# diff7/tts-king

Measured on AMD Instinct MI355X. Metric: FS2 train mel-frames/sec/GPU + HiFi-GAN RTF (22.05 kHz), batch=16, higher is better.
Workload: dtype bf16

## Files before the change

### tts_king_amd/csrc/batchnorm.hip

```cpp
#include "common.h"

namespace {

struct BnCommon {
  const void* x;
  const float* mean;
  const float* rstd;
  const float* gamma;
  const float* beta;
  const uint64_t* rng;
  int rows, C, use_tanh;
  float p;
  unsigned site;
  int x_f32;
  const int* frame_limit;
  int seg_len;
  uint8_t* keep;
  const long long* lens;
};
__device__ __forceinline__ float tanh_fast(float x) { return 1.f - 2.f * __frcp_rn(__expf(2.f * x) + 1.f); }
__device__ __forceinline__ bool bn_live(const int* frame_limit, int seg_len, int r) {
  return !frame_limit || (r % seg_len) < frame_limit[0];
}
__device__ __forceinline__ int bn_rows(const int* frame_limit, int seg_len, int rows) {
// ... 204 lines not shown
  if (blockIdx.x == 0 && dgamma)
    for (int c = threadIdx.x; c < a.C; c += 256) {
      dbeta[c] = accumulate ? dbeta[c] + sums[c] : sums[c];
      dgamma[c] = accumulate ? dgamma[c] + sums[a.C + c] : sums[a.C + c];
    }
  for (int64_t i = blockIdx.x * 256 + threadIdx.x; i < n; i += (int64_t)gridDim.x * 256) {
    const int r = (int)(i / tpr), c4 = (int)(i - (int64_t)r * tpr) * 4;
    float xh[4], dy[4];
    bn_dy(a, dout, dout_f32, r, c4, i, thr, scale, xh, dy);
    const f32x4 g = *(const f32x4*)(a.gamma + c4), rs = *(const f32x4*)(a.rstd + c4);
    const f32x4 s1 = *(const f32x4*)(sums + c4), s2 = *(const f32x4*)(sums + a.C + c4);
    float o[4];
#pragma unroll
    for (int e = 0; e < 4; ++e) o[e] = g[e] * rs[e] * (dy[e] - s1[e] * inv_n - xh[e] * s2[e] * inv_n);
    if (!bn_live(a.frame_limit, a.seg_len, r)) o[0] = o[1] = o[2] = o[3] = 0.f;
    *(uint2*)(dx + (int64_t)r * a.C + c4) = make_uint2(pack_bf2(o[0], o[1]), pack_bf2(o[2], o[3]));
  }
}


constexpr int BN_MAX_CHUNKS = 64;
__host__ __device__ inline int bn_slab(int C) { return (C % 64 == 0) ? 64 : C; }

struct BnSlab {
  int c0, slab, tpr, rpi, r_in, cq, rb, re;
  __device__ BnSlab(int C, int rows) {
    slab = bn_slab(C);
    c0 = blockIdx.x * slab;
    tpr = slab >> 2;
    rpi = 256 / tpr;
    r_in = threadIdx.x / tpr;
    cq = threadIdx.x % tpr;
    const int per = (rows + gridDim.y - 1) / gridDim.y;
    rb = blockIdx.y * per;
    re = min(rb + per, rows);
  }
};

__device__ __forceinline__ void bn_slab_store(const BnSlab& g, int C, const float s[4], const float q[4], float* red, float* partials) {
  if (g.r_in < g.rpi) {
#pragma unroll
    for (int e = 0; e < 4; ++e) { red[g.r_in * g.slab + g.cq * 4 + e] = s[e]; red[(g.rpi + g.r_in) * g.slab + g.cq * 4 + e] = q[e]; }
  }
  __syncthreads();
  for (int v = threadIdx.x; v < 2 * g.slab; v += 256) {
    const int half = v >= g.slab, c = v - half * g.slab;
    float acc = 0.f;
    for (int k = 0; k < g.rpi; ++k) acc += red[(half * g.rpi + k) * g.slab + c];
    partials[(int64_t)blockIdx.y * 2 * C + half * C + g.c0 + c] = acc;
  }
}

constexpr int BN_TOT = 256 + 1024;
__device__ __forceinline__ void bn_slab_totals(const float* __restrict__ partials, int nblk, int C, int c0, int slab, double* tot ) {
  const int nq = slab >> 1, groups = 256 / nq;
  const int t = threadIdx.x;
  if (t < groups * nq) {
    const int q = t % nq, g0 = t / nq;
    const int v0 = q * 4;
    const int col = v0 < slab ? c0 + v0 : C + c0 + (v0 - slab);
    double a[4] = {0.0, 0.0, 0.0, 0.0};
    for (int b = g0; b < nblk; b += 16 * groups) {
      f32x4 f[16];
#pragma unroll
      for (int u = 0; u < 16; ++u) {
        const int bb = b + u * groups;
        f[u] = *(const f32x4*)(partials + (int64_t)min(bb, nblk - 1) * 2 * C + col);
        if (bb >= nblk) f[u] = f32x4{0.f, 0.f, 0.f, 0.f};
      }
#pragma unroll
      for (int u = 0; u < 16; ++u)
#pragma unroll
        for (int e = 0; e < 4; ++e) a[e] += f[u][e];
    }
#pragma unroll
    for (int e = 0; e < 4; ++e) tot[256 + t * 4 + e] = a[e];
  }
  __syncthreads();
  if (t < 2 * slab) {
    double sum = 0.0;
    for (int k = 0; k < groups; ++k) sum += tot[256 + (k * nq + (t >> 2)) * 4 + (t & 3)];
    tot[t] = sum;
  }
  __syncthreads();
}

__global__ __launch_bounds__(256) void bn_stats2_kernel(const void* __restrict__ x, int x_f32, int rows, int C, float* __restrict__ partials,
                                                        const int* __restrict__ frame_limit, int seg_len) {
  extern __shared__ float red[];
  const BnSlab g(C, rows);
  const int c4 = g.c0 + g.cq * 4;
  float s[4] = {0, 0, 0, 0}, q[4] = {0, 0, 0, 0};
  if (g.r_in < g.rpi)
    for (int r0 = g.rb + g.r_in; r0 < g.re; r0 += 8 * g.rpi) {
      float v[8][4];
#pragma unroll
      for (int u = 0; u < 8; ++u) {
        const int r = r0 + u * g.rpi, rc = min(r, g.re - 1);
        ldx4(x, x_f32, (int64_t)rc * C + c4, v[u]);
        if (r >= g.re || !bn_live(frame_limit, seg_len, rc)) v[u][0] = v[u][1] = v[u][2] = v[u][3] = 0.f;
      }
#pragma unroll
      for (int u = 0; u < 8; ++u)
#pragma unroll
        for (int e = 0; e < 4; ++e) { s[e] += v[u][e]; q[e] += v[u][e] * v[u][e]; }
    }
  bn_slab_store(g, C, s, q, red, partials);
}

struct BnTrain {
  const float* partials;
  int nblk;
  float eps, momentum;
  float* mean;
  float* rstd;
  float* run_mean;
  float* run_var;
  long long* nbt;
};

template <bool RESID>
__global__ __launch_bounds__(256, RESID ? 3 : 4) void bn_apply2_kernel(const BnCommon a, const BnTrain t, const float* __restrict__ resid,
                                                        bf16_t* __restrict__ out16, float* __restrict__ out32) {
  __shared__ double tot[BN_TOT];
  __shared__ float ms[128], rs[128];
  const BnSlab g(a.C, a.rows);
  const int cl = g.cq * 4, c4 = g.c0 + cl, tprC = a.C >> 2;
  const bool act = g.r_in < g.rpi;
  float v[4][4], rr[RESID ? 4 : 1][4];
  bool live[4];
#pragma unroll
  for (int u = 0; u < 4; ++u) {
    const int r = g.rb + g.r_in + u * g.rpi, rc = max(min(r, g.re - 1), 0);
    live[u] = act && r < g.re && bn_live(a.frame_limit, a.seg_len, r);
    if (act) {
      ldx4(a.x, a.x_f32, (int64_t)rc * a.C + c4, v[u]);
      if constexpr (RESID) { const f32x4 q = *(const f32x4*)(resid + (int64_t)rc * a.C + c4); rr[u][0] = q[0]; rr[u][1] = q[1]; rr[u][2] = q[2]; rr[u][3] = q[3]; }
    }
  }
  f32x4 gm = f32x4{0.f, 0.f, 0.f, 0.f}, bt = gm;
  if (act) { gm = *(const f32x4*)(a.gamma + c4); bt = *(const f32x4*)(a.beta + c4); }
  bn_slab_totals(t.partials, t.nblk, a.C, g.c0, g.slab, tot);
  if ((int)threadIdx.x < g.slab) {
    const int c = threadIdx.x;
    const int n = bn_rows(a.frame_limit, a.seg_len, a.rows);
    const double m = tot[c] / n;
    double var = tot[g.slab + c] / n - m * m;
    if (var < 0.0) var = 0.0;
    ms[c] = (float)m;
    rs[c] = (float)(1.0 / sqrt(var + (double)t.eps));
    if (blockIdx.y == 0) {
      t.mean[g.c0 + c] = ms[c];
      t.rstd[g.c0 + c] = rs[c];
      if (t.run_mean) {
        t.run_mean[g.c0 + c] = (1.f - t.momentum) * t.run_mean[g.c0 + c] + t.momentum * (float)m;
        t.run_var[g.c0 + c] = (1.f - t.momentum) * t.run_var[g.c0 + c] + t.momentum * (float)(var * n / (n > 1 ? n - 1 : 1));
      }
      if (blockIdx.x == 0 && c == 0 && t.nbt) t.nbt[0] += 1;
    }
  }
  __syncthreads();
  if (!act) return;
  const unsigned thr = keep_threshold(a.p);
  const float scale = a.p > 0.f ? 1.f / (1.f - a.p) : 1.f;
#pragma unroll
  for (int u = 0; u < 4; ++u) {
    const int r = g.rb + g.r_in + u * g.rpi;
    if (r >= g.re) break;
    const int64_t i = (int64_t)r * tprC + (c4 >> 2);
    if (!live[u]) {
      if (out16) *(uint2*)(out16 + (int64_t)r * a.C + c4) = make_uint2(0u, 0u);
      if (out32) *(f32x4*)(out32 + (int64_t)r * a.C + c4) = f32x4{0.f, 0.f, 0.f, 0.f};
      if (a.keep) a.keep[i] = 0;
      continue;
    }
#pragma unroll
    for (int e = 0; e < 4; ++e) {
      v[u][e] = (v[u][e] - ms[cl + e]) * rs[cl + e] * gm[e] + bt[e];
      if (a.use_tanh) v[u][e] = tanh_fast(v[u][e]);
    }
    if (a.p > 0.f) {
      const unsigned nib = bn_keep4(a.rng, a.site, (unsigned)i, thr);
      drop4(v[u], nib, scale);
      if (a.keep) a.keep[i] = (uint8_t)nib;
    }
    if constexpr (RESID) {
#pragma unroll
      for (int e = 0; e < 4; ++e) v[u][e] += rr[u][e];
    }
    if (out16) *(uint2*)(out16 + (int64_t)r * a.C + c4) = make_uint2(pack_bf2(v[u][0], v[u][1]), pack_bf2(v[u][2], v[u][3]));
    if (out32) *(f32x4*)(out32 + (int64_t)r * a.C + c4) = f32x4{v[u][0], v[u][1], v[u][2], v[u][3]};
  }
}

__global__ __launch_bounds__(256) void bn_bwd_stats2_kernel(const BnCommon a, const void* __restrict__ dout, int dout_f32,
                                                            float* __restrict__ partials) {
  extern __shared__ float red[];
  const BnSlab g(a.C, a.rows);
  const int c4 = g.c0 + g.cq * 4, tprC = a.C >> 2;
  const unsigned thr = keep_threshold(a.p);
  const float scale = a.p > 0.f ? 1.f / (1.f - a.p) : 1.f;
  float s[4] = {0, 0, 0, 0}, q[4] = {0, 0, 0, 0};
  if (g.r_in < g.rpi)
    for (int r0 = g.rb + g.r_in; r0 < g.re; r0 += 8 * g.rpi) {
      float xh[8][4], dy[8][4];
#pragma unroll
      for (int u = 0; u < 8; ++u) {
        const int r = r0 + u * g.rpi, rc = min(r, g.re - 1);
        bn_dy(a, dout, dout_f32, rc, c4, (int64_t)rc * tprC + (c4 >> 2), thr, scale, xh[u], dy[u]);
        if (r >= g.re) { xh[u][0] = xh[u][1] = xh[u][2] = xh[u][3] = 0.f; dy[u][0] = dy[u][1] = dy[u][2] = dy[u][3] = 0.f; }
      }
#pragma unroll
      for (int u = 0; u < 8; ++u)
#pragma unroll
        for (int e = 0; e < 4; ++e) { s[e] += dy[u][e]; q[e] += dy[u][e] * xh[u][e]; }
    }
  bn_slab_store(g, a.C, s, q, red, partials);
}

__global__ __launch_bounds__(256, 4) void bn_bwd_apply2_kernel(const BnCommon a, const void* __restrict__ dout, int dout_f32,
                                                            const float* __restrict__ partials, int nblk, bf16_t* __restrict__ dx,
                                                            float* __restrict__ dgamma, float* __restrict__ dbeta, int accumulate) {
  __shared__ double tot[BN_TOT];
  __shared__ float s1s[128], s2s[128];
  const BnSlab g(a.C, a.rows);
  const int cl = g.cq * 4, c4 = g.c0 + cl, tprC = a.C >> 2;
  const bool act = g.r_in < g.rpi;
  const unsigned thr = keep_threshold(a.p);
  const float scale = a.p > 0.f ? 1.f / (1.f - a.p) : 1.f;
  float xh[4][4], dy[4][4];
#pragma unroll
  for (int u = 0; u < 4; ++u) {
    const int rc = max(min(g.rb + g.r_in + u * g.rpi, g.re - 1), 0);
    if (act) bn_dy(a, dout, dout_f32, rc, c4, (int64_t)rc * tprC + (c4 >> 2), thr, scale, xh[u], dy[u]);
  }
  bn_slab_totals(partials, nblk, a.C, g.c0, g.slab, tot);
  if ((int)threadIdx.x < g.slab) {
    const int c = threadIdx.x;
    s1s[c] = (float)tot[c];
    s2s[c] = (float)tot[g.slab + c];
    if (blockIdx.y == 0 && dgamma) {
      dbeta[g.c0 + c] = accumulate ? dbeta[g.c0 + c] + s1s[c] : s1s[c];
      dgamma[g.c0 + c] = accumulate ? dgamma[g.c0 + c] + s2s[c] : s2s[c];
    }
  }
  __syncthreads();
  if (!act) return;
  const float inv_n = 1.f / bn_rows(a.frame_limit, a.seg_len, a.rows);
  const f32x4 gm = *(const f32x4*)(a.gamma + c4), rsd = *(const f32x4*)(a.rstd + c4);
#pragma unroll
  for (int u = 0; u < 4; ++u) {
    const int r = g.rb + g.r_in + u * g.rpi;
    if (r >= g.re) break;
    float o[4];
#pragma unroll
    for (int e = 0; e < 4; ++e) o[e] = gm[e] * rsd[e] * (dy[u][e] - s1s[cl + e] * inv_n - xh[u][e] * s2s[cl + e] * inv_n);
    if (!bn_live(a.frame_limit, a.seg_len, r)) o[0] = o[1] = o[2] = o[3] = 0.f;
    *(uint2*)(dx + (int64_t)r * a.C + c4) = make_uint2(pack_bf2(o[0], o[1]), pack_bf2(o[2], o[3]));
  }
}

inline int bn_chunks(int rows) { int n = (rows + 15) / 16; return n > BN_MAX_CHUNKS ? BN_MAX_CHUNKS : (n < 1 ? 1 : n); }
inline int bn_apply_chunks(int rows, int C) { const int rpi = 256 / (bn_slab(C) >> 2); int n = (rows + 4 * rpi - 1) / (4 * rpi); return n < 1 ? 1 : n; }

inline int bn_blocks(int rows) { int n = (rows + 15) / 16; return n > 1024 ? 1024 : (n < 1 ? 1 : n); }

}

extern "C" int ttsk_bn_nblocks(int rows) { return bn_blocks(rows); }

static int bn_check(int rows, int C) {
  TTSK_REQUIRE(rows > 0 && C >= 4 && C <= 1024 && (C & 3) == 0, "batchnorm: C must be a multiple of 4, <= 1024 (got %d)", C);
  return 0;
}

static int limit_check(const int32_t* frame_limit, int seg_len, int rows) {
  TTSK_REQUIRE(!frame_limit || (seg_len > 0 && rows % seg_len == 0), "batchnorm: frame_limit needs rows %% seg_len == 0");
  return 0;
}

extern "C" int ttsk_bn_stats(const void* x, int x_is_f32, int rows, int C, float* partials, const int32_t* frame_limit, int seg_len,
                             void* stream) {
  TTSK_REQUIRE(x && partials, "bn_stats: null pointer");
  if (int rc = limit_check(frame_limit, seg_len, rows)) return rc;
  if (int rc = bn_check(rows, C)) return rc;
  const int rpi = 256 / (C >> 2);
  hipLaunchKernelGGL(bn_stats_kernel, dim3(bn_blocks(rows)), dim3(256), 2 * rpi * C * sizeof(float), (hipStream_t)stream,
                     x, x_is_f32, rows, C, partials, frame_limit, seg_len > 0 ? seg_len : 1);
  TTSK_CHECK_LAUNCH();
  return TTSK_OK;
}

extern "C" int ttsk_bn_finalize(const float* partials, int nblk, int C, int rows, float eps, float momentum, float* mean,
                                float* rstd, float* running_mean, float* running_var, int64_t* num_batches_tracked,
                                const int32_t* frame_limit, int seg_len, void* stream) {
  if (int rc = limit_check(frame_limit, seg_len, rows)) return rc;
  TTSK_REQUIRE(partials && mean && rstd && nblk > 0, "bn_finalize: null pointer");
  TTSK_REQUIRE((running_mean == nullptr) == (running_var == nullptr), "bn_finalize: running stats come in pairs");
  hipLaunchKernelGGL(bn_finalize_kernel, dim3((C + 15) / 16), dim3(256), 0, (hipStream_t)stream, partials, nblk, C, rows, eps,
                     momentum, mean, rstd, running_mean, running_var, (long long*)num_batches_tracked, frame_limit, seg_len > 0 ? seg_len : 1);
  TTSK_CHECK_LAUNCH();
  return TTSK_OK;
}

extern "C" int ttsk_rsqrt_eps(const float* var, float eps, float* rstd, int n, void* stream) {
  TTSK_REQUIRE(var && rstd && n > 0, "rsqrt_eps: bad arguments");
  hipLaunchKernelGGL(rsqrt_eps_kernel, dim3((n + 255) / 256), dim3(256), 0, (hipStream_t)stream, var, eps, rstd, n);
  TTSK_CHECK_LAUNCH();
  return TTSK_OK;
}
// ... 20 lines not shown
  TTSK_REQUIRE(x && mean && rstd && gamma && beta && lens && (out_bf16 || out_f32), "bn_apply_lens: null pointer");
  TTSK_REQUIRE(seg_len > 0 && rows % seg_len == 0, "bn_apply_lens: rows %% seg_len != 0");
  if (int rc = bn_check(rows, C)) return rc;
  BnCommon a{x, mean, rstd, gamma, beta, nullptr, rows, C, use_tanh, 0.f, 0u, x_is_f32, nullptr, seg_len, nullptr, (const long long*)lens};
  int64_t n = (int64_t)rows * (C >> 2);
  int blocks = (int)((n + 255) / 256);
  if (blocks > 4096) blocks = 4096;
  hipLaunchKernelGGL(bn_apply_kernel<true>, dim3(blocks), dim3(256), 0, (hipStream_t)stream, a, resid_f32, (bf16_t*)out_bf16, out_f32);
  TTSK_CHECK_LAUNCH();
  return TTSK_OK;
}

extern "C" int ttsk_bn_bwd_stats(const void* dout, int dout_is_f32, const void* x, int x_is_f32, const float* mean, const float* rstd,
                                 const float* gamma, const float* beta, int rows, int C, int use_tanh, float p, uint32_t site,
                                 const uint64_t* rng, float* partials, const int32_t* frame_limit, int seg_len, void* stream) {
  if (int rc = limit_check(frame_limit, seg_len, rows)) return rc;
  TTSK_REQUIRE(dout && x && mean && rstd && gamma && beta && partials, "bn_bwd_stats: null pointer");
  TTSK_REQUIRE(p == 0.f || rng, "bn_bwd_stats: dropout needs rng");
  if (int rc = bn_check(rows, C)) return rc;
  BnCommon a{x, mean, rstd, gamma, beta, rng, rows, C, use_tanh, p, site, x_is_f32, frame_limit, seg_len > 0 ? seg_len : 1};
  const int rpi = 256 / (C >> 2);
  hipLaunchKernelGGL(bn_bwd_stats_kernel, dim3(bn_blocks(rows)), dim3(256), 2 * rpi * C * sizeof(float), (hipStream_t)stream, a,
                     dout, dout_is_f32, partials);
  TTSK_CHECK_LAUNCH();
  return TTSK_OK;
}

extern "C" int ttsk_bn_bwd_apply(const void* dout, int dout_is_f32, const void* x, int x_is_f32, const float* mean, const float* rstd,
                                 const float* gamma, const float* beta, int rows, int C, int use_tanh, float p, uint32_t site,
                                 const uint64_t* rng, const float* sums, void* dx_bf16, float* dgamma, float* dbeta, int accumulate,
                                 const int32_t* frame_limit, int seg_len, void* stream) {
  if (int rc = limit_check(frame_limit, seg_len, rows)) return rc;
  TTSK_REQUIRE(dout && x && mean && rstd && gamma && beta && sums && dx_bf16, "bn_bwd_apply: null pointer");
  TTSK_REQUIRE((dgamma == nullptr) == (dbeta == nullptr), "bn_bwd_apply: dgamma/dbeta come in pairs");
  if (int rc = bn_check(rows, C)) return rc;
  BnCommon a{x, mean, rstd, gamma, beta, rng, rows, C, use_tanh, p, site, x_is_f32, frame_limit, seg_len > 0 ? seg_len : 1};
  int64_t n = (int64_t)rows * (C >> 2);
  int blocks = (int)((n + 255) / 256);
  if (blocks > 4096) blocks = 4096;
  hipLaunchKernelGGL(bn_bwd_apply_kernel, dim3(blocks), dim3(256), 0, (hipStream_t)stream, a, dout, dout_is_f32, sums,
                     (bf16_t*)dx_bf16, dgamma, dbeta, accumulate);
  TTSK_CHECK_LAUNCH();
  return TTSK_OK;
}

static int bn2_check(int rows, int C) {
  if (int rc = bn_check(rows, C)) return rc;
  TTSK_REQUIRE(C % 64 == 0 || C <= 128, "batchnorm (slab path): C must be a multiple of 64 or <= 128 (got %d)", C);
  return 0;
}

extern "C" int ttsk_bn_nchunks(int rows) { return bn_chunks(rows); }

extern "C" int ttsk_bn_stats_slab(const void* x, int x_is_f32, int rows, int C, float* partials, const int32_t* frame_limit, int seg_len,
                                  void* stream) {
  TTSK_REQUIRE(x && partials, "bn_stats_slab: null pointer");
  if (int rc = limit_check(frame_limit, seg_len, rows)) return rc;
  if (int rc = bn2_check(rows, C)) return rc;
  const int slab = bn_slab(C), rpi = 256 / (slab >> 2);
  hipLaunchKernelGGL(bn_stats2_kernel, dim3(C / slab, bn_chunks(rows)), dim3(256), 2 * rpi * slab * sizeof(float), (hipStream_t)stream,
                     x, x_is_f32, rows, C, partials, frame_limit, seg_len > 0 ? seg_len : 1);
  TTSK_CHECK_LAUNCH();
  return TTSK_OK;
}

extern "C" int ttsk_bn_train_apply(const void* x, int x_is_f32, const float* partials, int nblk, float eps, float momentum, float* mean,
                                   float* rstd, float* running_mean, float* running_var, int64_t* num_batches_tracked,
                                   const float* gamma, const float* beta, int rows, int C, int use_tanh, float p, uint32_t site,
                                   const uint64_t* rng, const float* resid_f32, void* out_bf16, float* out_f32, uint8_t* keep_out,
                                   const int32_t* frame_limit, int seg_len, void* stream) {
  if (int rc = limit_check(frame_limit, seg_len, rows)) return rc;
  TTSK_REQUIRE(x && partials && nblk > 0 && mean && rstd && gamma && beta && (out_bf16 || out_f32), "bn_train_apply: null pointer");
  TTSK_REQUIRE((running_mean == nullptr) == (running_var == nullptr), "bn_train_apply: running stats come in pairs");
  TTSK_REQUIRE(p == 0.f || rng, "bn_train_apply: dropout needs rng");
  if (int rc = bn2_check(rows, C)) return rc;
  BnCommon a{x, nullptr, nullptr, gamma, beta, rng, rows, C, use_tanh, p, site, x_is_f32, frame_limit, seg_len > 0 ? seg_len : 1, keep_out};
  BnTrain t{partials, nblk, eps, momentum, mean, rstd, running_mean, running_var, (long long*)num_batches_tracked};
  const dim3 grid(C / bn_slab(C), bn_apply_chunks(rows, C));
  if (resid_f32) hipLaunchKernelGGL(bn_apply2_kernel<true>, grid, dim3(256), 0, (hipStream_t)stream, a, t, resid_f32, (bf16_t*)out_bf16, out_f32);
  else hipLaunchKernelGGL(bn_apply2_kernel<false>, grid, dim3(256), 0, (hipStream_t)stream, a, t, resid_f32, (bf16_t*)out_bf16, out_f32);
  TTSK_CHECK_LAUNCH();
  return TTSK_OK;
}

extern "C" int ttsk_bn_bwd_stats_slab(const void* dout, int dout_is_f32, const void* x, int x_is_f32, const float* mean, const float* rstd,
                                      const float* gamma, const float* beta, int rows, int C, int use_tanh, float p, uint32_t site,
                                      const uint64_t* rng, const uint8_t* keep, float* partials, const int32_t* frame_limit, int seg_len,
                                      void* stream) {
  if (int rc = limit_check(frame_limit, seg_len, rows)) return rc;
  TTSK_REQUIRE(dout && x && mean && rstd && gamma && beta && partials, "bn_bwd_stats_slab: null pointer");
  TTSK_REQUIRE(p == 0.f || rng || keep, "bn_bwd_stats_slab: dropout needs rng or the forward's keep bits");
  if (int rc = bn2_check(rows, C)) return rc;
  BnCommon a{x, mean, rstd, gamma, beta, rng, rows, C, use_tanh, p, site, x_is_f32, frame_limit, seg_len > 0 ? seg_len : 1, (uint8_t*)keep};
  const int slab = bn_slab(C), rpi = 256 / (slab >> 2);
  hipLaunchKernelGGL(bn_bwd_stats2_kernel, dim3(C / slab, bn_chunks(rows)), dim3(256), 2 * rpi * slab * sizeof(float), (hipStream_t)stream,
                     a, dout, dout_is_f32, partials);
  TTSK_CHECK_LAUNCH();
  return TTSK_OK;
}

extern "C" int ttsk_bn_bwd_apply_slab(const void* dout, int dout_is_f32, const void* x, int x_is_f32, const float* mean, const float* rstd,
                                      const float* gamma, const float* beta, int rows, int C, int use_tanh, float p, uint32_t site,
                                      const uint64_t* rng, const uint8_t* keep, const float* partials, int nblk, void* dx_bf16, float* dgamma,
                                      float* dbeta, int accumulate, const int32_t* frame_limit, int seg_len, void* stream) {
  if (int rc = limit_check(frame_limit, seg_len, rows)) return rc;
  TTSK_REQUIRE(dout && x && mean && rstd && gamma && beta && partials && nblk > 0 && dx_bf16, "bn_bwd_apply_slab: null pointer");
  TTSK_REQUIRE((dgamma == nullptr) == (dbeta == nullptr), "bn_bwd_apply_slab: dgamma/dbeta come in pairs");
  TTSK_REQUIRE(p == 0.f || rng || keep, "bn_bwd_apply_slab: dropout needs rng or the forward's keep bits");
  if (int rc = bn2_check(rows, C)) return rc;
  BnCommon a{x, mean, rstd, gamma, beta, rng, rows, C, use_tanh, p, site, x_is_f32, frame_limit, seg_len > 0 ? seg_len : 1, (uint8_t*)keep};
  hipLaunchKernelGGL(bn_bwd_apply2_kernel, dim3(C / bn_slab(C), bn_apply_chunks(rows, C)), dim3(256), 0, (hipStream_t)stream, a, dout,
                     dout_is_f32, partials, nblk, (bf16_t*)dx_bf16, dgamma, dbeta, accumulate);
  TTSK_CHECK_LAUNCH();
  return TTSK_OK;
}
```

### tts_king_amd/csrc/ffn_conv.hip

```cpp
#include "common.h"
#include "tapring.h"

namespace {

constexpr int WC_H = 4, WC_NW = 8, WC_NT = WC_NW * 64, WC_KH = 4, WC_CT = 2, WC_COUT = WC_NW * WC_CT * 16;

struct WcArgs {
  const bf16_t* x;
  const bf16_t* w;
  const float* bias;
  void* out;
  int S, K, Cout, relu;
  int B, tiles_per_utt;
  const bf16_t* gate;
  int nsplit, ldx;
  int64_t out_split;
  const float* o32;
  float* delta;
  float* stats;
  const int* frame_limit;
  int ups_cout;
  int ups_half;
  const float* bnb_x;
  const float* bnb_mean;
// ... 136 lines not shown
  {
    const int id = blockIdx.x, ncg = (a.Cout / COUT) * a.nsplit, ntile = a.tiles_per_utt * a.B;
    const int xcd = id & 7, per = 8 / (ncg < 8 ? ncg : 8);
    int tile;
    if ((8 % (ncg < 8 ? ncg : 8)) == 0 && ncg <= 8 && (ntile * ncg) % 8 == 0 && ntile % per == 0) {
      cg = xcd / per;
      tile = (id >> 3) * per + (xcd % per);
    } else if (ncg % 8 == 0) {
      const int gpx = ncg >> 3, slot = id >> 3;
      tile = slot / gpx;
      cg = xcd * gpx + (slot - tile * gpx);
    } else {
      cg = id / ntile;
      tile = id - cg * ntile;
    }
    bi = tile / a.tiles_per_utt;
    t0 = (tile - bi * a.tiles_per_utt) * TT;
    sp = cg % a.nsplit;
    cg = cg / a.nsplit;
  }
  WC_STAMP(0);
  const int S = a.S, K = a.K, HK = (K - 1) / 2, NS = NP * K;
  const int ldx = a.ldx;
  const bf16_t* __restrict__ xb = a.x + (int64_t)bi * S * ldx + sp * C;
  const bf16_t* __restrict__ wbase = a.w;
  const int ks_total = (ldx + 31) / 32, ks_base = sp * (C / 32);
  const int cin_valid = a.cin_valid > 0 ? a.cin_valid : C;

  const __amdgpu_buffer_rsrc_t wres = weights_rsrc(wbase, K * ks_total * 32 * a.Cout * 2);
  const int wlane = PACKED ? (cg * (COUT / 16) + wave * CT) * 1024 + lane * 16 : ((cg * COUT + wave * CT * 16 + l15) * K * C + q * 8) * 2;
  constexpr bool CAN_DIRECT = PACKED && !F16 && CIN == 256 && TT == 112 && NWV == 8 && CTV == 2;
  const bool direct = CAN_DIRECT && a.direct;
  int wl[CT];
#pragma unroll
  for (int cc = 0; cc < CT; ++cc) {
    const int co = 32 * wave + 8 * (l15 >> 2) + 4 * cc + (l15 & 3);
    wl[cc] = direct ? (cg * (COUT / 16) + (co >> 4)) * 1024 + ((co & 15) + 16 * q) * 16 : wlane + cc * 1024;
  }
  const int kstep_bytes = (a.Cout / 16) * 1024;
  bf16x8 wa[KH][CT], wb[KH][CT], wc[KH][CT];
  auto load_w = [&](int g, bf16x8 (&w)[KH][CT]) __attribute__((always_inline)) {
    const int tap = g / NP, part = g - tap * NP;
    if (PACKED) {
      frags_load<KH, CT>(w, wres, wl, (tap * ks_total + ks_base + part * KH) * kstep_bytes, kstep_bytes);
    } else {
      const int soff = (tap * C + part * (KH * 32)) * 2;
#pragma unroll
      for (int ks = 0; ks < KH; ++ks)
#pragma unroll
        for (int cc = 0; cc < CT; ++cc) w[ks][cc] = frag_load(wres, wlane, soff + ks * 64 + cc * (16 * K * C * 2));
    }
  };

  {
    constexpr int NCH = (XROWS * CH8 + NT - 1) / NT;
    uint4 xv[NCH];
#pragma unroll
    for (int it = 0; it < NCH; ++it) {
      const int idx = it * NT + tid;
      const int row = idx / CH8, ch = idx - row * CH8;
      const int t = t0 - WC_H + row;
      xv[it] = make_uint4(0, 0, 0, 0);
      if (idx < XROWS * CH8 && t >= 0 && t < S && ch * 8 < cin_valid) xv[it] = *(const uint4*)(xb + (int64_t)t * ldx + ch * 8);
    }
    load_w(0, wa);
    if (!F16 || 1 < NS) load_w(min(1, NS - 1), wb);
    if (!F16 || 2 < NS) load_w(min(2, NS - 1), wc);
#pragma unroll
    for (int it = 0; it < NCH; ++it) {
      const int idx = it * NT + tid;
      const int row = idx / CH8, ch = idx - row * CH8;
      if (idx < XROWS * CH8) *(uint4*)(XW + row * RS + ch * 16) = xv[it];
    }
  }
  f32x4 bv[CT];
#pragma unroll
  for (int cc = 0; cc < CT; ++cc)
    bv[cc] = a.bias ? *(const f32x4*)(a.bias + cg * COUT + (direct ? 32 * wave + 8 * q + 4 * cc : (wave * CT + cc) * 16 + q * 4)) : f32x4{0.f, 0.f, 0.f, 0.f};
  WC_STAMP(1);
  __syncthreads();
  WC_STAMP(2);

  f32x4 acc[CT][NF];
#pragma unroll
  for (int cc = 0; cc < CT; ++cc)
#pragma unroll
    for (int i = 0; i < NF; ++i) acc[cc][i] = f32x4{0.f, 0.f, 0.f, 0.f};
  {
    const int inl = (l15 + WC_H) * RS + q * 16;
    const int ups_shift = F16 && a.ups_cout ? ((cg * COUT + wave * CT * 16) / a.ups_cout < a.ups_half ? -1 : 1) : 0;
    constexpr bool RING = NF <= 8;
    auto inp_of = [&](int g) __attribute__((always_inline)) {
      const int tap = g / NP, part = g - tap * NP;
      return inl + (F16 && a.ups_cout ? tap * ups_shift : tap - HK) * RS + part * (KH * 64);
    };
    bf16x8 ring[RING ? NF : 1];
    if constexpr (RING) ring_prime<NF, RS>(ring, XW, inp_of(0));
    auto step = [&](int g, const bf16x8 (&w)[KH][CT]) __attribute__((always_inline)) {
      const int inp = inp_of(g);
      if constexpr (RING) {
        tap_ring<F16, KH, CT, NF, RS>(acc, ring, w, XW, inp, inp_of(g + 1 < NS ? g + 1 : g));
      } else {
#pragma unroll
        for (int ks = 0; ks < KH; ++ks) {
#pragma unroll
          for (int i = 0; i < NF; ++i) {
            const bf16x8 Bf = *(const bf16x8*)(XW + inp + i * 16 * RS + ks * 64);
#pragma unroll
            for (int cc = 0; cc < CT; ++cc) acc[cc][i] = mfma16<F16>(w[ks][cc], Bf, acc[cc][i]);
          }
        }
      }
    };
    constexpr bool UNCOND = !F16;
#pragma unroll 1
    for (int g = 0; g < NS; g += 3) {
      step(g, wa);
      if (UNCOND || g + 3 < NS) load_w(min(g + 3, NS - 1), wa);
      if (g + 1 < NS) step(g + 1, wb);
      if (UNCOND || g + 4 < NS) load_w(min(g + 4, NS - 1), wb);
      if (g + 2 < NS) step(g + 2, wc);
      if (UNCOND || g + 5 < NS) load_w(min(g + 5, NS - 1), wc);
    }
  }
  WC_STAMP(3);
#ifdef TTSK_STAMPS
  if (a.stamps && lane == 0 && wave < 8) {
    a.stamps[(int64_t)blockIdx.x * 24 + 8 + wave] = __builtin_amdgcn_s_memrealtime();
    a.stamps[(int64_t)blockIdx.x * 24 + 16 + wave] = __builtin_amdgcn_s_getreg(63492);
  }
#endif
// ... 548 lines not shown
```

### tts_king_amd/csrc/layernorm.hip

```cpp
#include "common.h"
#include "proj32.h"

namespace {

constexpr int MAXJ = 4;

struct LnArgs {
  const bf16_t* y;
  const bf16_t* res;
  const float* gamma;
  const float* beta;
  bf16_t* out;
  bf16_t* z_save;
  float* mean;
  float* rstd;
  const long long* lens;
  const uint64_t* rng;
  const float* head_w;
  const float* head_b;
  float* head_out;
  int rows, D, seg_len;
  float p_pre, p_post, eps;
  unsigned site_pre, site_post;
  int group_rows;
// ... 229 lines not shown
  }
  const int nq = head ? 4 : 3;
  float* P = a.partials + (int64_t)blockIdx.x * (nq * D + (head ? 1 : 0));
  for (int qn = 0; qn < nq; ++qn) {
#pragma unroll
    for (int j = 0; j < MJ; ++j)
      if (j < nj)
#pragma unroll
        for (int e = 0; e < 4; ++e) {
          const float v = qn == 0 ? dbias[j][e] : qn == 1 ? dg[j][e] : qn == 2 ? db[j][e] : dhw[j][e];
          red[wave][j * 256 + lane * 4 + e] = v;
        }
    __syncthreads();
    for (int c = threadIdx.x; c < D; c += LNB_WAVES * 64) {
      float t = 0.f;
#pragma unroll
      for (int w = 0; w < LNB_WAVES; ++w) t += red[w][c];
      P[qn * D + c] = t;
    }
    __syncthreads();
  }
  if (head) {
    dhb = wave_sum(dhb);
    if (lane == 0) redb[wave] = dhb;
    __syncthreads();
    if (threadIdx.x == 0) {
      float t = 0.f;
#pragma unroll
      for (int w = 0; w < LNB_WAVES; ++w) t += redb[w];
      P[nq * D] = t;
    }
  }
}

__device__ __forceinline__ void unpack8(uint4 u, float* v) {
  v[0] = __uint_as_float(u.x << 16); v[1] = __uint_as_float(u.x & 0xFFFF0000u);
  v[2] = __uint_as_float(u.y << 16); v[3] = __uint_as_float(u.y & 0xFFFF0000u);
  v[4] = __uint_as_float(u.z << 16); v[5] = __uint_as_float(u.z & 0xFFFF0000u);
  v[6] = __uint_as_float(u.w << 16); v[7] = __uint_as_float(u.w & 0xFFFF0000u);
}
__device__ __forceinline__ uint4 pack8f(const float* v) {
  return make_uint4(pack_bf2(v[0], v[1]), pack_bf2(v[2], v[3]), pack_bf2(v[4], v[5]), pack_bf2(v[6], v[7]));
}
__device__ __forceinline__ void hold(uint4& v) { asm volatile("" : "+v"(v.x), "+v"(v.y), "+v"(v.z), "+v"(v.w)); }
__device__ __forceinline__ void hold(f32x4& v) { asm volatile("" : "+v"(v)); }
__device__ __forceinline__ void hold(float& v) { asm volatile("" : "+v"(v)); }
__device__ __forceinline__ float group16_sum(float v) { return quad16_sum(v); }

__device__ __forceinline__ void lnb256_row(const LnBwdArgs& a, int row, int c0, const float gam[16], uint64_t seed, uint64_t step,
                                           unsigned thr, float dscale, float sbias[16], float sgam[16], float sbeta[16], float dzv[16],
                                           const float* dl = nullptr ) {
  constexpr int D = 256;
  const bool live = row < a.rows;
  bool masked = !live;
  if (live && a.lens) { const int b = row / a.seg_len, t = row - b * a.seg_len; masked = t >= a.lens[b]; }
  float zz[16], d[16];
#pragma unroll
  for (int e = 0; e < 16; ++e) { zz[e] = 0.f; d[e] = 0.f; }
  const bool slabbed = dl || a.slabs, use = live && !masked;
  const int64_t ro = (int64_t)(live ? row : a.rows - 1) * D + c0;
  uint4 zr[2] = {*(const uint4*)(a.z + ro), *(const uint4*)(a.z + ro + 8)};
  float mean = a.mean[live ? row : a.rows - 1], rstd = a.rstd[live ? row : a.rows - 1];
  const float* sp = a.slabs ? a.slabs + ro : nullptr;
  const bool slab0 = !dl && a.slabs && a.nsplit > 0;
  f32x4 s0[4];
  if (dl) {
#pragma unroll
    for (int i = 0; i < 4; ++i) s0[i] = *(const f32x4*)(dl + c0 + 4 * i);
  } else {
    const float* s0p = slab0 ? sp : a.gamma + c0;
#pragma unroll
    for (int i = 0; i < 4; ++i) s0[i] = *(const f32x4*)(s0p + 4 * i);
  }
  const bf16_t* up = slabbed ? (a.R ? a.R : a.z) : a.dout;
  uint4 ur[2] = {*(const uint4*)(up + ro), *(const uint4*)(up + ro + 8)};
  __builtin_amdgcn_sched_barrier(0);
  unsigned kb = 0;
  if (a.p_pre > 0.f) {
#pragma unroll
    for (int i = 0; i < 4; ++i) kb |= keep4(seed, step, a.site_pre, (unsigned)(((int64_t)row * D + c0 + 4 * i) >> 2), thr) << (4 * i);
  }
  __builtin_amdgcn_sched_barrier(0);
  hold(zr[0]); hold(zr[1]); hold(mean); hold(rstd); hold(ur[0]); hold(ur[1]);
#pragma unroll
  for (int i = 0; i < 4; ++i) hold(s0[i]);
  if (!live) { mean = 0.f; rstd = 0.f; }
  if (live) { unpack8(zr[0], zz); unpack8(zr[1], zz + 8); }
  if (use) {
    if (slabbed) {
      if (dl) {
#pragma unroll
        for (int i = 0; i < 4; ++i) { d[4 * i] = s0[i][0]; d[4 * i + 1] = s0[i][1]; d[4 * i + 2] = s0[i][2]; d[4 * i + 3] = s0[i][3]; }
      } else {
        if (slab0) {
#pragma unroll
          for (int i = 0; i < 4; ++i) { d[4 * i] += s0[i][0]; d[4 * i + 1] += s0[i][1]; d[4 * i + 2] += s0[i][2]; d[4 * i + 3] += s0[i][3]; }
        }
        for (int q = 1; q < a.nsplit; ++q) {
#pragma unroll
          for (int i = 0; i < 4; ++i) {
            const f32x4 t = *(const f32x4*)(sp + q * a.slab_stride + 4 * i);
            d[4 * i] += t[0]; d[4 * i + 1] += t[1]; d[4 * i + 2] += t[2]; d[4 * i + 3] += t[3];
          }
        }
      }
      if (a.R) {
        float r[16];
        unpack8(ur[0], r); unpack8(ur[1], r + 8);
#pragma unroll
        for (int e = 0; e < 16; ++e) d[e] += r[e];
      }
    } else {
      unpack8(ur[0], d); unpack8(ur[1], d + 8);
    }
  }
  float xh[16], g[16];
  float c1 = 0.f, c2 = 0.f;
#pragma unroll
  for (int e = 0; e < 16; ++e) {
    xh[e] = __fmul_rn(__fsub_rn(zz[e], mean), rstd);
    g[e] = __fmul_rn(d[e], gam[e]);
    c1 = __fadd_rn(c1, g[e]); c2 = __fmaf_rn(g[e], xh[e], c2);
    sgam[e] = __fmaf_rn(d[e], xh[e], sgam[e]);
    sbeta[e] = __fadd_rn(sbeta[e], d[e]);
  }
  c1 = __fmul_rn(group16_sum(c1), 1.f / D);
  c2 = __fmul_rn(group16_sum(c2), 1.f / D);
#pragma unroll
  for (int e = 0; e < 16; ++e) dzv[e] = __fmul_rn(rstd, __fmaf_rn(-xh[e], c2, __fsub_rn(g[e], c1)));
  if (live && a.dz) {
    bf16_t* op = a.dz + (int64_t)row * D + c0;
    *(uint4*)op = pack8f(dzv); *(uint4*)(op + 8) = pack8f(dzv + 8);
  }
  if (a.p_pre > 0.f) {
#pragma unroll
    for (int i = 0; i < 4; ++i) drop4(dzv + 4 * i, kb >> (4 * i), dscale);
    if (live && a.dy) {
      bf16_t* op = a.dy + (int64_t)row * D + c0;
// ... 665 lines not shown
```

Baseline: 2.535 million.

## Issue BN/conv/LN global loads early and specialize BN kernels by dtype

BatchNorm apply and backward kernels now issue their x, dout, keep-mask and partial-sum loads before any conditional logic, holding them in registers with asm barriers so their latency overlaps the dropout RNG and stats reduction. The kernels are templated on input dtype and dropout mode, which removes runtime branches. The FFN conv and LayerNorm backward use clamped unconditional loads (bias, x tile, lens) with masking applied afterwards, so the loads are not gated by branches. The cost is higher register pressure, more template instantiations, and dummy reads from clamped or substitute addresses.

```diff
diff --git a/tts_king_amd/csrc/batchnorm.hip b/tts_king_amd/csrc/batchnorm.hip
--- a/tts_king_amd/csrc/batchnorm.hip
+++ b/tts_king_amd/csrc/batchnorm.hip
@@ -280,21 +280,42 @@
 }
 
 constexpr int BN_TOT = 256 + 1024;
-__device__ __forceinline__ void bn_slab_totals(const float* __restrict__ partials, int nblk, int C, int c0, int slab, double* tot ) {
-  const int nq = slab >> 1, groups = 256 / nq;
+struct BnPart {
+  int nq, groups, q, g0, col;
+  __device__ BnPart(int C, int c0, int slab) {
+    nq = slab >> 1;
+    groups = 256 / nq;
+    q = threadIdx.x % nq;
+    g0 = threadIdx.x / nq;
+    const int v0 = q * 4;
+    col = v0 < slab ? c0 + v0 : C + c0 + (v0 - slab);
+  }
+};
+__device__ __forceinline__ void bn_slab_request(const float* __restrict__ partials, int nblk, int C, const BnPart& pt, f32x4 f[16]) {
+#pragma unroll
+  for (int u = 0; u < 16; ++u) f[u] = *(const f32x4*)(partials + (int64_t)min(pt.g0 + u * pt.groups, nblk - 1) * 2 * C + pt.col);
+}
+template <bool HOLD>
+__device__ __forceinline__ void bn_slab_totals(const float* __restrict__ partials, int nblk, int C, int slab, const BnPart& pt, const f32x4 f0[16],
+                                               double* tot ) {
+  const int nq = pt.nq, groups = pt.groups;
   const int t = threadIdx.x;
   if (t < groups * nq) {
-    const int q = t % nq, g0 = t / nq;
-    const int v0 = q * 4;
-    const int col = v0 < slab ? c0 + v0 : C + c0 + (v0 - slab);
     double a[4] = {0.0, 0.0, 0.0, 0.0};
-    for (int b = g0; b < nblk; b += 16 * groups) {
+#pragma unroll
+    for (int u = 0; u < 16; ++u) {
+      const f32x4 fu = pt.g0 + u * groups < nblk ? f0[u] : f32x4{0.f, 0.f, 0.f, 0.f};
+#pragma unroll
+      for (int e = 0; e < 4; ++e) a[e] += fu[e];
+    }
+    for (int b = pt.g0 + 16 * groups; b < nblk; b += 16 * groups) {
       f32x4 f[16];
 #pragma unroll
+      for (int u = 0; u < 16; ++u) f[u] = *(const f32x4*)(partials + (int64_t)min(b + u * groups, nblk - 1) * 2 * C + pt.col);
+#pragma unroll
       for (int u = 0; u < 16; ++u) {
-        const int bb = b + u * groups;
-        f[u] = *(const f32x4*)(partials + (int64_t)min(bb, nblk - 1) * 2 * C + col);
-        if (bb >= nblk) f[u] = f32x4{0.f, 0.f, 0.f, 0.f};
+        if constexpr (HOLD) asm volatile("" : "+v"(f[u]));
+        if (b + u * groups >= nblk) f[u] = f32x4{0.f, 0.f, 0.f, 0.f};
       }
 #pragma unroll
       for (int u = 0; u < 16; ++u)
@@ -312,6 +333,66 @@
   }
   __syncthreads();
 }
+
+template <bool F32> struct BnRaw;
+template <> struct BnRaw<true> {
+  f32x4 r;
+  __device__ __forceinline__ void request(const void* p, int64_t off) { r = *(const f32x4*)((const float*)p + off); }
+  __device__ __forceinline__ void hold() { asm volatile("" : "+v"(r)); }
+  __device__ __forceinline__ void unpack(float v[4]) const { v[0] = r[0]; v[1] = r[1]; v[2] = r[2]; v[3] = r[3]; }
+};
+template <> struct BnRaw<false> {
+  uint2 r;
+  __device__ __forceinline__ void request(const void* p, int64_t off) { r = *(const uint2*)((const bf16_t*)p + off); }
+  __device__ __forceinline__ void hold() { asm volatile("" : "+v"(r.x), "+v"(r.y)); }
+  __device__ __forceinline__ void unpack(float v[4]) const {
+    v[0] = __uint_as_float(r.x << 16); v[1] = __uint_as_float(r.x & 0xFFFF0000u);
+    v[2] = __uint_as_float(r.y << 16); v[3] = __uint_as_float(r.y & 0xFFFF0000u);
+  }
+};
+struct BnLimit {
+  int lim, seg_len;
+  bool on;
+  __device__ __forceinline__ BnLimit(const BnCommon& a) {
+    on = a.frame_limit != nullptr;
+    const int v = *(on ? a.frame_limit : (const int*)a.gamma);
+    lim = on ? v : 0x7FFFFFFF;
+    seg_len = a.seg_len;
+  }
+  __device__ __forceinline__ bool live(int r) const { return (r % seg_len) < lim; }
+  __device__ __forceinline__ int rows(int rows_all) const { return on ? (rows_all / seg_len) * lim : rows_all; }
+};
+template <bool XF32, bool DF32, bool DRAW> struct BnBwdRow {
+  BnRaw<XF32> x;
+  BnRaw<DF32> d;
+  unsigned kb;
+  __device__ __forceinline__ void request(const BnCommon& a, const void* dout, const uint8_t* kp, int r, int c4, int64_t i) {
+    x.request(a.x, (int64_t)r * a.C + c4);
+    d.request(dout, (int64_t)r * a.C + c4);
+    if constexpr (!DRAW) kb = kp[i];
+  }
+  __device__ __forceinline__ void hold() {
+    x.hold(); d.hold();
+    if constexpr (!DRAW) asm volatile("" : "+v"(kb));
+  }
+  __device__ __forceinline__ void math(const BnCommon& a, const f32x4& m, const f32x4& rs, const f32x4& g, const f32x4& b, float scale,
+                                       bool live, float xh[4], float dy[4]) const {
+    float v[4];
+    x.unpack(v);
+    d.unpack(dy);
+    if (a.p > 0.f) drop4(dy, kb, scale);
+#pragma unroll
+    for (int e = 0; e < 4; ++e) xh[e] = (v[e] - m[e]) * rs[e];
+    if (a.use_tanh) {
+#pragma unroll
+      for (int e = 0; e < 4; ++e) { const float t = tanh_fast(xh[e] * g[e] + b[e]); dy[e] *= 1.f - t * t; }
+    }
+    if (!live) {
+#pragma unroll
+      for (int e = 0; e < 4; ++e) { xh[e] = 0.f; dy[e] = 0.f; }
+    }
+  }
+};
 
 __global__ __launch_bounds__(256) void bn_stats2_kernel(const void* __restrict__ x, int x_f32, int rows, int C, float* __restrict__ partials,
                                                         const int* __restrict__ frame_limit, int seg_len) {
@@ -347,31 +428,37 @@
   long long* nbt;
 };
 
-template <bool RESID>
+template <bool RESID, bool XF32>
 __global__ __launch_bounds__(256, RESID ? 3 : 4) void bn_apply2_kernel(const BnCommon a, const BnTrain t, const float* __restrict__ resid,
                                                         bf16_t* __restrict__ out16, float* __restrict__ out32) {
   __shared__ double tot[BN_TOT];
   __shared__ float ms[128], rs[128];
+  const BnLimit fl(a);
   const BnSlab g(a.C, a.rows);
   const int cl = g.cq * 4, c4 = g.c0 + cl, tprC = a.C >> 2;
   const bool act = g.r_in < g.rpi;
-  float v[4][4], rr[RESID ? 4 : 1][4];
+  BnRaw<XF32> xr[4];
+  f32x4 rr[RESID ? 4 : 1];
+#pragma unroll
+  for (int u = 0; u < 4; ++u) {
+    const int rc = max(min(g.rb + g.r_in + u * g.rpi, g.re - 1), 0);
+    xr[u].request(a.x, (int64_t)rc * a.C + c4);
+    if constexpr (RESID) rr[u] = *(const f32x4*)(resid + (int64_t)rc * a.C + c4);
+  }
+  f32x4 gm = *(const f32x4*)(a.gamma + c4), bt = *(const f32x4*)(a.beta + c4);
+  const BnPart pt(a.C, g.c0, g.slab);
+  f32x4 pf[16];
+  bn_slab_request(t.partials, t.nblk, a.C, pt, pf);
   bool live[4];
 #pragma unroll
   for (int u = 0; u < 4; ++u) {
-    const int r = g.rb + g.r_in + u * g.rpi, rc = max(min(r, g.re - 1), 0);
-    live[u] = act && r < g.re && bn_live(a.frame_limit, a.seg_len, r);
-    if (act) {
-      ldx4(a.x, a.x_f32, (int64_t)rc * a.C + c4, v[u]);
-      if constexpr (RESID) { const f32x4 q = *(const f32x4*)(resid + (int64_t)rc * a.C + c4); rr[u][0] = q[0]; rr[u][1] = q[1]; rr[u][2] = q[2]; rr[u][3] = q[3]; }
-    }
-  }
-  f32x4 gm = f32x4{0.f, 0.f, 0.f, 0.f}, bt = gm;
-  if (act) { gm = *(const f32x4*)(a.gamma + c4); bt = *(const f32x4*)(a.beta + c4); }
-  bn_slab_totals(t.partials, t.nblk, a.C, g.c0, g.slab, tot);
+    const int r = g.rb + g.r_in + u * g.rpi;
+    live[u] = act && r < g.re && fl.live(r);
+  }
+  bn_slab_totals<true>(t.partials, t.nblk, a.C, g.slab, pt, pf, tot);
   if ((int)threadIdx.x < g.slab) {
     const int c = threadIdx.x;
-    const int n = bn_rows(a.frame_limit, a.seg_len, a.rows);
+    const int n = fl.rows(a.rows);
     const double m = tot[c] / n;
     double var = tot[g.slab + c] / n - m * m;
     if (var < 0.0) var = 0.0;
@@ -402,41 +489,65 @@
       if (a.keep) a.keep[i] = 0;
       continue;
     }
+    float v[4];
+    xr[u].unpack(v);
 #pragma unroll
     for (int e = 0; e < 4; ++e) {
-      v[u][e] = (v[u][e] - ms[cl + e]) * rs[cl + e] * gm[e] + bt[e];
-      if (a.use_tanh) v[u][e] = tanh_fast(v[u][e]);
+      v[e] = (v[e] - ms[cl + e]) * rs[cl + e] * gm[e] + bt[e];
+      if (a.use_tanh) v[e] = tanh_fast(v[e]);
     }
     if (a.p > 0.f) {
       const unsigned nib = bn_keep4(a.rng, a.site, (unsigned)i, thr);
-      drop4(v[u], nib, scale);
+      drop4(v, nib, scale);
       if (a.keep) a.keep[i] = (uint8_t)nib;
     }
     if constexpr (RESID) {
 #pragma unroll
-      for (int e = 0; e < 4; ++e) v[u][e] += rr[u][e];
-    }
-    if (out16) *(uint2*)(out16 + (int64_t)r * a.C + c4) = make_uint2(pack_bf2(v[u][0], v[u][1]), pack_bf2(v[u][2], v[u][3]));
-    if (out32) *(f32x4*)(out32 + (int64_t)r * a.C + c4) = f32x4{v[u][0], v[u][1], v[u][2], v[u][3]};
-  }
-}
-
-__global__ __launch_bounds__(256) void bn_bwd_stats2_kernel(const BnCommon a, const void* __restrict__ dout, int dout_f32,
-                                                            float* __restrict__ partials) {
+      for (int e = 0; e < 4; ++e) v[e] += rr[u][e];
+    }
+    if (out16) *(uint2*)(out16 + (int64_t)r * a.C + c4) = make_uint2(pack_bf2(v[0], v[1]), pack_bf2(v[2], v[3]));
+    if (out32) *(f32x4*)(out32 + (int64_t)r * a.C + c4) = f32x4{v[0], v[1], v[2], v[3]};
+  }
+}
+
+template <int N, bool XF32, bool DF32, bool DRAW>
+__device__ __forceinline__ void bn_bwd_draw_hold(const BnCommon& a, BnBwdRow<XF32, DF32, DRAW> (&row)[N], const int64_t (&idx)[N], unsigned thr) {
+  if constexpr (DRAW) {
+#pragma unroll
+    for (int u = 0; u < N; ++u) row[u].kb = bn_keep4(a.rng, a.site, (unsigned)idx[u], thr);
+  }
+#pragma unroll
+  for (int u = 0; u < N; ++u) row[u].hold();
+}
+
+template <bool XF32, bool DF32, bool DRAW>
+__global__ __launch_bounds__(256) void bn_bwd_stats2_kernel(const BnCommon a, const void* __restrict__ dout, float* __restrict__ partials) {
   extern __shared__ float red[];
+  const BnLimit fl(a);
   const BnSlab g(a.C, a.rows);
   const int c4 = g.c0 + g.cq * 4, tprC = a.C >> 2;
   const unsigned thr = keep_threshold(a.p);
   const float scale = a.p > 0.f ? 1.f / (1.f - a.p) : 1.f;
+  const uint8_t* kp = a.keep ? a.keep : (const uint8_t*)a.x;
+  const f32x4 cm = *(const f32x4*)(a.mean + c4), crs = *(const f32x4*)(a.rstd + c4);
+  const f32x4 cg = *(const f32x4*)(a.gamma + c4), cb = *(const f32x4*)(a.beta + c4);
   float s[4] = {0, 0, 0, 0}, q[4] = {0, 0, 0, 0};
   if (g.r_in < g.rpi)
     for (int r0 = g.rb + g.r_in; r0 < g.re; r0 += 8 * g.rpi) {
+      BnBwdRow<XF32, DF32, DRAW> row[8];
+      int64_t idx[8];
+#pragma unroll
+      for (int u = 0; u < 8; ++u) {
+        const int rc = min(r0 + u * g.rpi, g.re - 1);
+        idx[u] = (int64_t)rc * tprC + (c4 >> 2);
+        row[u].request(a, dout, kp, rc, c4, idx[u]);
+      }
+      bn_bwd_draw_hold(a, row, idx, thr);
       float xh[8][4], dy[8][4];
 #pragma unroll
       for (int u = 0; u < 8; ++u) {
-        const int r = r0 + u * g.rpi, rc = min(r, g.re - 1);
-        bn_dy(a, dout, dout_f32, rc, c4, (int64_t)rc * tprC + (c4 >> 2), thr, scale, xh[u], dy[u]);
-        if (r >= g.re) { xh[u][0] = xh[u][1] = xh[u][2] = xh[u][3] = 0.f; dy[u][0] = dy[u][1] = dy[u][2] = dy[u][3] = 0.f; }
+        const int r = r0 + u * g.rpi;
+        row[u].math(a, cm, crs, cg, cb, scale, r < g.re && fl.live(r), xh[u], dy[u]);
       }
 #pragma unroll
       for (int u = 0; u < 8; ++u)
@@ -446,23 +557,43 @@
   bn_slab_store(g, a.C, s, q, red, partials);
 }
 
-__global__ __launch_bounds__(256, 4) void bn_bwd_apply2_kernel(const BnCommon a, const void* __restrict__ dout, int dout_f32,
+template <bool XF32, bool DF32, bool DRAW>
+__global__ __launch_bounds__(256, 4) void bn_bwd_apply2_kernel(const BnCommon a, const void* __restrict__ dout,
                                                             const float* __restrict__ partials, int nblk, bf16_t* __restrict__ dx,
                                                             float* __restrict__ dgamma, float* __restrict__ dbeta, int accumulate) {
   __shared__ double tot[BN_TOT];
   __shared__ float s1s[128], s2s[128];
+  const BnLimit fl(a);
   const BnSlab g(a.C, a.rows);
   const int cl = g.cq * 4, c4 = g.c0 + cl, tprC = a.C >> 2;
   const bool act = g.r_in < g.rpi;
   const unsigned thr = keep_threshold(a.p);
   const float scale = a.p > 0.f ? 1.f / (1.f - a.p) : 1.f;
-  float xh[4][4], dy[4][4];
+  const uint8_t* kp = a.keep ? a.keep : (const uint8_t*)a.x;
+  BnBwdRow<XF32, DF32, DRAW> row[4];
+  int64_t idx[4];
 #pragma unroll
   for (int u = 0; u < 4; ++u) {
     const int rc = max(min(g.rb + g.r_in + u * g.rpi, g.re - 1), 0);
-    if (act) bn_dy(a, dout, dout_f32, rc, c4, (int64_t)rc * tprC + (c4 >> 2), thr, scale, xh[u], dy[u]);
-  }
-  bn_slab_totals(partials, nblk, a.C, g.c0, g.slab, tot);
+    idx[u] = (int64_t)rc * tprC + (c4 >> 2);
+    row[u].request(a, dout, kp, rc, c4, idx[u]);
+  }
+  const f32x4 cm = *(const f32x4*)(a.mean + c4), rsd = *(const f32x4*)(a.rstd + c4);
+  const f32x4 gm = *(const f32x4*)(a.gamma + c4), cb = *(const f32x4*)(a.beta + c4);
+  bn_bwd_draw_hold(a, row, idx, thr);
+  float xh[4][4], dy[4][4];
+#pragma unroll
+  for (int u = 0; u < 4; ++u) {
+    const int rc = max(min(g.rb + g.r_in + u * g.rpi, g.re - 1), 0);
+    row[u].math(a, cm, rsd, gm, cb, scale, fl.live(rc), xh[u], dy[u]);
+  }
+  float gr[4];
+#pragma unroll
+  for (int e = 0; e < 4; ++e) gr[e] = gm[e] * rsd[e];
+  const BnPart pt(a.C, g.c0, g.slab);
+  f32x4 pf[16];
+  bn_slab_request(partials, nblk, a.C, pt, pf);
+  bn_slab_totals<false>(partials, nblk, a.C, g.slab, pt, pf, tot);
   if ((int)threadIdx.x < g.slab) {
     const int c = threadIdx.x;
     s1s[c] = (float)tot[c];
@@ -474,16 +605,15 @@
   }
   __syncthreads();
   if (!act) return;
-  const float inv_n = 1.f / bn_rows(a.frame_limit, a.seg_len, a.rows);
-  const f32x4 gm = *(const f32x4*)(a.gamma + c4), rsd = *(const f32x4*)(a.rstd + c4);
+  const float inv_n = 1.f / fl.rows(a.rows);
 #pragma unroll
   for (int u = 0; u < 4; ++u) {
     const int r = g.rb + g.r_in + u * g.rpi;
     if (r >= g.re) break;
     float o[4];
 #pragma unroll
-    for (int e = 0; e < 4; ++e) o[e] = gm[e] * rsd[e] * (dy[u][e] - s1s[cl + e] * inv_n - xh[u][e] * s2s[cl + e] * inv_n);
-    if (!bn_live(a.frame_limit, a.seg_len, r)) o[0] = o[1] = o[2] = o[3] = 0.f;
+    for (int e = 0; e < 4; ++e) o[e] = gr[e] * (dy[u][e] - s1s[cl + e] * inv_n - xh[u][e] * s2s[cl + e] * inv_n);
+    if (!fl.live(r)) o[0] = o[1] = o[2] = o[3] = 0.f;
     *(uint2*)(dx + (int64_t)r * a.C + c4) = make_uint2(pack_bf2(o[0], o[1]), pack_bf2(o[2], o[3]));
   }
 }
@@ -610,6 +740,10 @@
 
 extern "C" int ttsk_bn_nchunks(int rows) { return bn_chunks(rows); }
 
+#define BN_BWD_INSTANCE(K, XF, DF, DRAW)                                                                    \
+  ((XF) ? ((DF) ? ((DRAW) ? K<true, true, true> : K<true, true, false>) : ((DRAW) ? K<true, false, true> : K<true, false, false>)) \
+        : ((DF) ? ((DRAW) ? K<false, true, true> : K<false, true, false>) : ((DRAW) ? K<false, false, true> : K<false, false, false>)))
+
 extern "C" int ttsk_bn_stats_slab(const void* x, int x_is_f32, int rows, int C, float* partials, const int32_t* frame_limit, int seg_len,
                                   void* stream) {
   TTSK_REQUIRE(x && partials, "bn_stats_slab: null pointer");
@@ -635,8 +769,9 @@
   BnCommon a{x, nullptr, nullptr, gamma, beta, rng, rows, C, use_tanh, p, site, x_is_f32, frame_limit, seg_len > 0 ? seg_len : 1, keep_out};
   BnTrain t{partials, nblk, eps, momentum, mean, rstd, running_mean, running_var, (long long*)num_batches_tracked};
   const dim3 grid(C / bn_slab(C), bn_apply_chunks(rows, C));
-  if (resid_f32) hipLaunchKernelGGL(bn_apply2_kernel<true>, grid, dim3(256), 0, (hipStream_t)stream, a, t, resid_f32, (bf16_t*)out_bf16, out_f32);
-  else hipLaunchKernelGGL(bn_apply2_kernel<false>, grid, dim3(256), 0, (hipStream_t)stream, a, t, resid_f32, (bf16_t*)out_bf16, out_f32);
+  auto* kern = resid_f32 ? (x_is_f32 ? bn_apply2_kernel<true, true> : bn_apply2_kernel<true, false>)
+                         : (x_is_f32 ? bn_apply2_kernel<false, true> : bn_apply2_kernel<false, false>);
+  hipLaunchKernelGGL(kern, grid, dim3(256), 0, (hipStream_t)stream, a, t, resid_f32, (bf16_t*)out_bf16, out_f32);
   TTSK_CHECK_LAUNCH();
   return TTSK_OK;
 }
@@ -651,8 +786,8 @@
   if (int rc = bn2_check(rows, C)) return rc;
   BnCommon a{x, mean, rstd, gamma, beta, rng, rows, C, use_tanh, p, site, x_is_f32, frame_limit, seg_len > 0 ? seg_len : 1, (uint8_t*)keep};
   const int slab = bn_slab(C), rpi = 256 / (slab >> 2);
-  hipLaunchKernelGGL(bn_bwd_stats2_kernel, dim3(C / slab, bn_chunks(rows)), dim3(256), 2 * rpi * slab * sizeof(float), (hipStream_t)stream,
-                     a, dout, dout_is_f32, partials);
+  hipLaunchKernelGGL(BN_BWD_INSTANCE(bn_bwd_stats2_kernel, x_is_f32, dout_is_f32, p > 0.f && !keep), dim3(C / slab, bn_chunks(rows)), dim3(256),
+                     2 * rpi * slab * sizeof(float), (hipStream_t)stream, a, dout, partials);
   TTSK_CHECK_LAUNCH();
   return TTSK_OK;
 }
@@ -667,8 +802,8 @@
   TTSK_REQUIRE(p == 0.f || rng || keep, "bn_bwd_apply_slab: dropout needs rng or the forward's keep bits");
   if (int rc = bn2_check(rows, C)) return rc;
   BnCommon a{x, mean, rstd, gamma, beta, rng, rows, C, use_tanh, p, site, x_is_f32, frame_limit, seg_len > 0 ? seg_len : 1, (uint8_t*)keep};
-  hipLaunchKernelGGL(bn_bwd_apply2_kernel, dim3(C / bn_slab(C), bn_apply_chunks(rows, C)), dim3(256), 0, (hipStream_t)stream, a, dout,
-                     dout_is_f32, partials, nblk, (bf16_t*)dx_bf16, dgamma, dbeta, accumulate);
-  TTSK_CHECK_LAUNCH();
-  return TTSK_OK;
-}
+  hipLaunchKernelGGL(BN_BWD_INSTANCE(bn_bwd_apply2_kernel, x_is_f32, dout_is_f32, p > 0.f && !keep), dim3(C / bn_slab(C), bn_apply_chunks(rows, C)),
+                     dim3(256), 0, (hipStream_t)stream, a, dout, partials, nblk, (bf16_t*)dx_bf16, dgamma, dbeta, accumulate);
+  TTSK_CHECK_LAUNCH();
+  return TTSK_OK;
+}
diff --git a/tts_king_amd/csrc/ffn_conv.hip b/tts_king_amd/csrc/ffn_conv.hip
--- a/tts_king_amd/csrc/ffn_conv.hip
+++ b/tts_king_amd/csrc/ffn_conv.hip
@@ -212,16 +212,31 @@
     }
   };
 
+  f32x4 bv[CT];
+  constexpr bool BRANCHY = F16 || CTV != 1 || (CIN == 256 && NWV == 5);
   {
     constexpr int NCH = (XROWS * CH8 + NT - 1) / NT;
     uint4 xv[NCH];
+    auto inside = [&](int idx, int row, int ch) __attribute__((always_inline)) {
+      const int t = t0 - WC_H + row;
+      return idx < XROWS * CH8 && t >= 0 && t < S && ch * 8 < cin_valid;
+    };
 #pragma unroll
     for (int it = 0; it < NCH; ++it) {
       const int idx = it * NT + tid;
       const int row = idx / CH8, ch = idx - row * CH8;
-      const int t = t0 - WC_H + row;
-      xv[it] = make_uint4(0, 0, 0, 0);
-      if (idx < XROWS * CH8 && t >= 0 && t < S && ch * 8 < cin_valid) xv[it] = *(const uint4*)(xb + (int64_t)t * ldx + ch * 8);
+      if constexpr (BRANCHY) {
+        xv[it] = make_uint4(0, 0, 0, 0);
+        if (inside(idx, row, ch)) xv[it] = *(const uint4*)(xb + (int64_t)(t0 - WC_H + row) * ldx + ch * 8);
+      } else {
+        const int tc = max(min(t0 - WC_H + row, S - 1), 0);
+        xv[it] = *(const uint4*)(xb + (int64_t)tc * ldx + (inside(idx, row, ch) ? ch * 8 : 0));
+      }
+    }
+    if constexpr (!BRANCHY) {
+#pragma unroll
+      for (int cc = 0; cc < CT; ++cc)
+        bv[cc] = *(const f32x4*)(a.bias ? a.bias + cg * COUT + (direct ? 32 * wave + 8 * q + 4 * cc : (wave * CT + cc) * 16 + q * 4) : (const float*)wbase);
     }
     load_w(0, wa);
     if (!F16 || 1 < NS) load_w(min(1, NS - 1), wb);
@@ -230,13 +245,22 @@
     for (int it = 0; it < NCH; ++it) {
       const int idx = it * NT + tid;
       const int row = idx / CH8, ch = idx - row * CH8;
+      if constexpr (!BRANCHY) {
+        asm volatile("" : "+v"(xv[it].x), "+v"(xv[it].y), "+v"(xv[it].z), "+v"(xv[it].w));
+        if (!inside(idx, row, ch)) xv[it] = make_uint4(0, 0, 0, 0);
+      }
       if (idx < XROWS * CH8) *(uint4*)(XW + row * RS + ch * 16) = xv[it];
     }
   }
-  f32x4 bv[CT];
-#pragma unroll
-  for (int cc = 0; cc < CT; ++cc)
-    bv[cc] = a.bias ? *(const f32x4*)(a.bias + cg * COUT + (direct ? 32 * wave + 8 * q + 4 * cc : (wave * CT + cc) * 16 + q * 4)) : f32x4{0.f, 0.f, 0.f, 0.f};
+#pragma unroll
+  for (int cc = 0; cc < CT; ++cc) {
+    if constexpr (BRANCHY) {
+      bv[cc] = a.bias ? *(const f32x4*)(a.bias + cg * COUT + (direct ? 32 * wave + 8 * q + 4 * cc : (wave * CT + cc) * 16 + q * 4)) : f32x4{0.f, 0.f, 0.f, 0.f};
+    } else {
+      asm volatile("" : "+v"(bv[cc]));
+      if (!a.bias) bv[cc] = f32x4{0.f, 0.f, 0.f, 0.f};
+    }
+  }
   WC_STAMP(1);
   __syncthreads();
   WC_STAMP(2);
diff --git a/tts_king_amd/csrc/layernorm.hip b/tts_king_amd/csrc/layernorm.hip
--- a/tts_king_amd/csrc/layernorm.hip
+++ b/tts_king_amd/csrc/layernorm.hip
@@ -305,13 +305,14 @@
                                            const float* dl = nullptr ) {
   constexpr int D = 256;
   const bool live = row < a.rows;
-  bool masked = !live;
-  if (live && a.lens) { const int b = row / a.seg_len, t = row - b * a.seg_len; masked = t >= a.lens[b]; }
   float zz[16], d[16];
 #pragma unroll
   for (int e = 0; e < 16; ++e) { zz[e] = 0.f; d[e] = 0.f; }
-  const bool slabbed = dl || a.slabs, use = live && !masked;
-  const int64_t ro = (int64_t)(live ? row : a.rows - 1) * D + c0;
+  const int rowc = live ? row : a.rows - 1, seg = a.lens ? a.seg_len : 1;
+  const int ub = rowc / seg, ut = rowc - ub * seg;
+  long long ulen = (a.lens ? a.lens : (const long long*)a.gamma)[a.lens ? ub : 0];
+  const bool slabbed = dl || a.slabs;
+  const int64_t ro = (int64_t)rowc * D + c0;
   uint4 zr[2] = {*(const uint4*)(a.z + ro), *(const uint4*)(a.z + ro + 8)};
   float mean = a.mean[live ? row : a.rows - 1], rstd = a.rstd[live ? row : a.rows - 1];
   const float* sp = a.slabs ? a.slabs + ro : nullptr;
@@ -337,6 +338,8 @@
   hold(zr[0]); hold(zr[1]); hold(mean); hold(rstd); hold(ur[0]); hold(ur[1]);
 #pragma unroll
   for (int i = 0; i < 4; ++i) hold(s0[i]);
+  asm volatile("" : "+v"(ulen));
+  const bool masked = !live || (a.lens && ut >= ulen), use = live && !masked;
   if (!live) { mean = 0.f; rstd = 0.f; }
   if (live) { unpack8(zr[0], zz); unpack8(zr[1], zz + 8); }
   if (use) {
```

New measurement: 2.555 million, median of 6. About the same (+0.8%).
